# MycroftAI/mimic3

Hardware: AMD Instinct MI355X
Metric: 22.05 kHz audio samples/sec/node (en_UK/apope_low VITS hot path: run + int16, host ids in -> host int16 out) (higher is better)
Workload: dtype f32 (dense convs: operands split exactly into 3 x bf16, 6 bf16-MFMA products per multiply-add, f32 accumulate; f32 in / f32 out, parity at the f32 tolerances)

## Files before the change

### mimic3_amd/csrc/engine.cpp

```cpp
#include "engine.h"

#include <algorithm>
#include <cmath>
#include <cstdlib>
#include <cstring>
#include <fstream>
#include <sstream>

namespace m355 {

namespace {
struct Reader {
    const unsigned char* p;
    size_t n, pos = 0;
    void need(size_t k) const {
        if (pos + k > n) throw EngineError(MI355VITS_ERR_FORMAT, "weight container truncated");
    }
    template <typename T> T get() {
        need(sizeof(T));
        T v;
        memcpy(&v, p + pos, sizeof(T));
        pos += sizeof(T);
        return v;
    }
// ... 1080 lines not shown
        conv("convflow.proj", cw(p + ".proj"), a);
        {
            ProfScope ps(prof_, "spline");
            launch_spline_inverse(d_z2_, ch0, d_theta_, d_len_, B, Tx, c.dp_num_bins, c.dp_tail_bound,
                                  1.0f / sqrtf((float)H), stream_);
        }
    }
    ch0 ^= 1;
    {
        ProfScope ps(prof_, "durations");
        launch_durations(d_z2_, ch0, model_->ea_m[0], model_->ea_logs[0], d_len_, d_forced_, B, Tx, d_scales_, d_logw_, d_wceil_,
                         d_cum_, d_ylen_, stream_);
    }
    tap("logw", d_logw_, {B, 1, Tx});
}

static const char* stage_label(int i, const char* const (&t)[4]) { return t[std::min(i, 3)]; }

void Engine::coupling_layer(int j, int B, int Ty) {
    const mi355vits_config& c = cfg_;
    const int H = c.hidden_channels, I = c.inter_channels, half = I / 2;
    const long zbs = (long)I * Ty, hbs = (long)H * Ty;
    const bool rev = ((c.flow_n_flows - 1 - j) % 2) == 0;
    float* x0 = d_z_ + (rev ? (long)half * Ty : 0);
    float* x1 = d_z_ + (rev ? 0 : (long)half * Ty);
    ConvArgs pre;
    pre.x = x0; pre.x_bs = zbs; pre.x_ld = Ty;
    pre.y = d_fh_; pre.y_bs = hbs; pre.y_ld = Ty;
    pre.out_len = d_ylen_;
    pre.B = B; pre.T = Ty;
    conv("flow.pre", cw(S("flow.%d.pre", j)), pre);
    float* hcur = d_fh_;
    float* hnext = d_fh2_;
    for (int l = 0; l < c.flow_wn_layers; ++l) {
        int dil = 1;
        for (int q = 0; q < l; ++q) dil *= c.flow_wn_dilation_rate;
        const ConvW& win = cw(S("flow.%d.in.%d", j, l));
        const ConvW& wrs = cw(S("flow.%d.rs.%d", j, l));
        const float* cond_l = d_cond_flow_.empty() ? nullptr : d_cond_flow_[j] + (long)l * 2 * H;
        const bool wn_b3 = sw_.wn_b3 && math_on_bf16(kmath()) && win.packed_b3s != NO_OFF && wrs.packed_b3s != NO_OFF &&
                           conv1d_b3_supported(win.Cin, win.Cout, win.K, dil, Ty) && !sw_.force_generic;
        const bool fused = !sw_.force_generic && !sw_.no_fused_wn && !wn_b3;
        const bool b3 = fused && math_on_bf16(kmath()) && win.packed_b3w != NO_OFF && wrs.packed_b3s != NO_OFF &&
                        wn_layer_b3_supported(H, win.K, dil);
        if (b3 || (fused && wn_layer_fused_supported(H, win.K, dil))) {
            const bool h2 = b3 && math_ == MATH_F16X2 && win.packed_h2s != NO_OFF && wrs.packed_h2s != NO_OFF;
            WnArgs w;
            w.h_in = hcur; w.h_out = hnext; w.h_bs = hbs; w.h_ld = Ty;
            w.skip = d_fskip_; w.s_bs = hbs; w.s_ld = Ty;
            w.w_in = P(h2 ? win.packed_h2s : (b3 ? win.packed_b3w : win.packed)); w.b_in = P(win.bias);
            w.w_rs = P(h2 ? wrs.packed_h2s : (b3 ? wrs.packed_b3s : wrs.packed)); w.b_rs = P(wrs.bias);
            w.cond = cond_l; w.cond_bs = 2L * H * c.flow_wn_layers;
            w.len = d_ylen_;
            w.B = B; w.H = H; w.T = Ty; w.K = win.K; w.dil = dil; w.Crs = wrs.Cout; w.skip_init = (l == 0);
            if (b3) w.math = h2 ? (int)MATH_F16X2 : kmath();
            const double fl = 2.0 * B * (double)Ty * H * ((double)win.Cout * win.K + wrs.Cout);
            ProfScope ps(prof_, b3 ? "flow.wn_layer_b3" : "flow.wn_layer", fl, 4.0 * B * (double)Ty * H * 4);
            if (b3) launch_wn_layer_b3(w, stream_);
            else launch_wn_layer(w, stream_);
            if (wrs.Cout == 2 * H) std::swap(hcur, hnext);
            continue;
        }
        ConvArgs in;
        in.x = hcur; in.x_bs = hbs; in.x_ld = Ty;
        in.y = d_fu_; in.y_bs = hbs; in.y_ld = Ty;
        in.epi = EPI_GATE; in.H = H; in.dil = dil;
        if (cond_l) {
            in.cond = cond_l;
            in.cond_bs = 2L * H * c.flow_wn_layers;
        }
        in.B = B; in.T = Ty;
        if (wn_b3) in.math = kmath();
        conv("flow.in_gate", win, in);
        ConvArgs rs;
        rs.x = d_fu_; rs.x_bs = hbs; rs.x_ld = Ty;
        rs.y = hcur; rs.y_bs = hbs; rs.y_ld = Ty;
        rs.y2 = d_fskip_; rs.y2_bs = hbs; rs.y2_ld = Ty;
        rs.epi = EPI_RESSKIP; rs.H = H; rs.skip_init = (l == 0);
        rs.out_len = d_ylen_;
        rs.B = B; rs.T = Ty;
        if (wn_b3) rs.math = kmath();
        conv("flow.res_skip", wrs, rs);
    }
    ConvArgs post;
    post.x = d_fskip_; post.x_bs = hbs; post.x_ld = Ty;
    post.y = x1; post.y_bs = zbs; post.y_ld = Ty;
    post.res = x1; post.res_bs = zbs; post.res_ld = Ty; post.res_sub = 1;
    post.in_len = d_ylen_; post.out_len = d_ylen_;
    post.B = B; post.T = Ty;
    conv("flow.post_couple", cw(S("flow.%d.post", j)), post);
}

ConvArgs Engine::rb2_conv_args(int i, int j, int m, int B, int ch, long T) const {
    const mi355vits_config& c = cfg_;
    float* const pp[2] = {d_bufB_, d_bufT_};
    const bool last = (m == c.resblock_n_dilations[j] - 1);
    const float* src = m == 0 ? d_bufA_ : pp[(m - 1) & 1];
    ConvArgs a;
    a.x = src; a.x_bs = (long)ch * T; a.x_ld = (int)T;
    a.y = last ? d_bufC_ : pp[m & 1]; a.y_bs = (long)ch * T; a.y_ld = (int)T;
    a.res = src; a.res_bs = (long)ch * T; a.res_ld = (int)T;
    a.in_slope = 0.1f; a.dil = c.resblock_dilations[j * MI355VITS_MAX_STAGES + m];
    a.in_len = d_slen_ + (long)(i + 1) * B;
    if (last) { a.out_scale = 1.0f / c.n_resblock_kernels; a.accumulate = (j > 0); }
    a.B = B; a.T = (int)T;
    return a;
// ... 450 lines not shown
```

### mimic3_amd/csrc/kernels.h

```cpp
#pragma once
#include "hipx.h"

#include <vector>

namespace m355 {

struct Profiler;

enum ConvEpilogue { EPI_STD = 0, EPI_GATE = 1, EPI_RESSKIP = 2 };

struct ConvArgs {
    const float* x = nullptr; long x_bs = 0; int x_ld = 0;
    float* y = nullptr;       long y_bs = 0; int y_ld = 0;
    const float* w = nullptr;
    const float* wb3 = nullptr;
    int math = 0;
    const float* bias = nullptr;
    const float* cond = nullptr; long cond_bs = 0;
    const float* res = nullptr; long res_bs = 0; int res_ld = 0;
    float* y2 = nullptr; long y2_bs = 0; int y2_ld = 0;
    const int* in_len = nullptr;
    const int* in_len_host = nullptr;
    int nvalid = 0;
    int rb_loop = 0;
// ... 67 lines not shown
    const float* bias[MRF_MAX_RB][2] = {};
    int k[MRF_MAX_RB] = {}, d1[MRF_MAX_RB] = {}, d2[MRF_MAX_RB] = {};
    int nrb = 0;
    const int* len = nullptr;
    int B = 1, C = 0, T = 0;
    int R = 0, ldx = 0, ld1 = 0, vec = 0;
    float out_scale = 0.0f;
    int ablate = 0;
    int seg = 0;
    unsigned* clk = nullptr;
    const int* len_host = nullptr;
    int nvalid = 0;
    int prio = 0;
};
bool mrf_fused_supported(int C, int nrb, const int* k, const int* d1, const int* d2);
void launch_mrf_fused(MrfArgs a, hipStream_t s);
inline int mrf_stage_halo(int nrb, const int* k, const int* d1, const int* d2) {
    int R = 0;
    for (int j = 0; j < nrb; ++j) {
        const int r = (k[j] - 1) / 2 * d1[j] + (k[j] - 1) / 2 * d2[j];
        R = R > r ? R : r;
    }
    return R;
}
struct MrfPlan { int width = 0, halo = 0, x_ring = 0, x1_ring = 0; };
bool mrf_fused_plan(int C, int nrb, const int* k, const int* d1, const int* d2, MrfPlan* out);
bool mrf_p_plan(int C, int nrb, const int* k, const int* d1, const int* d2, MrfPlan* out);
bool mrf_s_plan(int C, int nrb, const int* k, const int* d1, const int* d2, MrfPlan* out);
size_t p16_packed_words(int Cout, int Cin, int K);
void pack_conv_weights_p16(const float* w, int Cout, int Cin, int K, uint32_t* out);
bool mrf_p_supported(int C, int nrb, const int* k, const int* d1, const int* d2);
int mrf_valid_items(const int* len_host, const int* len_dev, int B, int T, int block, int extra = 0);
void launch_mrf_p(MrfArgs a, hipStream_t s);
bool mrf_s_supported(int C, int nrb, const int* k, const int* d1, const int* d2);
int mrf_s_segment(int C, int B, int T, int cus, const int* len_host = nullptr);
void launch_mrf_s(MrfArgs a, hipStream_t s);
bool rb_conv_supported(const ConvArgs& a);
void launch_rb_conv(ConvArgs a, hipStream_t s);
void pack_conv_weights_p16n(const float* w, int Cout, int Cin, int K, uint32_t* out);
bool ups_pl_supported(const ConvArgs& a);
void launch_ups_pl(ConvArgs a, hipStream_t s);
int current_device_cu_count();
void set_max_dynamic_lds(const void* fn, int bytes);

struct WnArgs {
    const float* h_in = nullptr; float* h_out = nullptr; long h_bs = 0; int h_ld = 0;
    float* skip = nullptr; long s_bs = 0; int s_ld = 0;
    const float* w_in = nullptr;
    const float* b_in = nullptr;
    const float* w_rs = nullptr;
    const float* b_rs = nullptr;
    const float* cond = nullptr; long cond_bs = 0;
    const int* len = nullptr;
    int B = 1, H = 0, T = 0, K = 1, dil = 1, Crs = 0, skip_init = 0;
    int ldx = 0, vec = 0;
    int ablate = 0;
    int math = 0;
};
bool wn_layer_fused_supported(int H, int K, int dil);
void launch_wn_layer(WnArgs a, hipStream_t s);
bool wn_layer_b3_supported(int H, int K, int dil);
void launch_wn_layer_b3(WnArgs a, hipStream_t s);
int wn_layer_b3_column_tiles(const WnArgs& a);
int wn_layer_geometry(const WnArgs& a);

void launch_conv_post_tanh(const float* x, long x_bs, int x_ld, const float* w, int Cin, int K, int B, int L,
                           const int* valid_len, float* audio, long audio_bs, unsigned* peak_bits, hipStream_t s);
void launch_pcm16(const float* audio, long audio_bs, const unsigned* peak_bits, const int* valid_len, int B, int L,
                  int16_t* pcm, long pcm_bs, hipStream_t s, const double* volumes = nullptr);
enum PackEncoding { PACK_ENC_S16 = 0, PACK_ENC_ULAW = 1, PACK_ENC_ALAW = 2, PACK_ENC_F32 = 3 };
constexpr int pack_bytes_per_sample(int enc) { return enc == PACK_ENC_S16 ? 2 : enc == PACK_ENC_F32 ? 4 : 1; }
inline size_t pack_capacity_bytes(int enc, long total) { return ((size_t)total * pack_bytes_per_sample(enc) + 15) & ~size_t(15); }
enum { PACK_SEG_OFFSET = 0, PACK_SEG_ROW = 1, PACK_SEG_LENGTH = 2, PACK_SEG_SKIP = 3 };
constexpr int pack_seg_scale_row(bool trimmed) { return trimmed ? 4 : 3; }
constexpr int pack_seg_rows(bool trimmed, bool normalised) { return pack_seg_scale_row(trimmed) + (normalised ? 1 : 0); }
constexpr int pack_seg_curve_row(bool trimmed) { return pack_seg_scale_row(trimmed) + 1; }
constexpr int pack_seg_rows(bool trimmed, bool normalised, bool curved) { return pack_seg_rows(trimmed, normalised) + (curved ? 1 : 0); }
void launch_pack(int enc, const float* audio, long audio_bs, const unsigned* peak_bits, const double* volumes, const int* seg, int n,
                 uint8_t* out, long total, hipStream_t s, bool trimmed, bool normalised, const float* curve = nullptr);
enum { PACK_ENT_OFFSET = 0, PACK_ENT_ROW = 1, PACK_ENT_LENGTH = 2, PACK_ENT_SKIP = 3, PACK_ENT_ENC = 4, PACK_ENT_SCALE = 5, PACK_ENT_ROWS = 6 };
enum { PACK_ENT_SCALED = 4, PACK_ENT_CURVED = 8 };
enum { PACK_ENT_CURVE = 6 };
constexpr int pack_ent_rows(bool curved) { return curved ? PACK_ENT_ROWS + 1 : PACK_ENT_ROWS; }
enum { PACK_STREAM_BEGIN = 0, PACK_STREAM_DATA = 1, PACK_STREAM_END = 2, PACK_STREAM_ENC = 3, PACK_STREAM_HEADER = 4, PACK_STREAM_WORDS = 20 };
constexpr long PACK_STREAMS_ITEM_BYTES = 256L * 16;
inline size_t pack_streams_capacity(long n_bytes) { return ((size_t)n_bytes + 15) & ~size_t(15); }
inline size_t pack_streams_table_words(int n_entries, int n_streams, bool curved = false) {
    return (size_t)pack_ent_rows(curved) * n_entries + (size_t)PACK_STREAM_WORDS * n_streams;
}
void launch_pack_streams(const float* audio, long audio_bs, const unsigned* peak_bits, const double* volumes, const int* tab, int n_entries,
                         int n_streams, uint8_t* out, long n_bytes, hipStream_t s, const float* curve = nullptr);
void launch_g711_encode(int law, const int16_t* in, long n, uint8_t* out, hipStream_t s);

constexpr int FLAC_BLOCK = 4096;
constexpr int FLAC_SLOT_BYTES = 8208;
constexpr int FLAC_HEADER_BYTES = 42;
constexpr int FLAC_MAX_RATE = 0xfffff;
constexpr long FLAC_MAX_FRAME_NUMBER = 0x1fffff;
struct FlacJob {
    const int16_t* src;
    long n;
    int first_frame;
    int slot0;
};
inline long flac_frames(long n) { return (n + FLAC_BLOCK - 1) / FLAC_BLOCK; }
inline size_t flac_out_capacity(long n_frames, long total) { return (16 * (size_t)n_frames + 2 * (size_t)total + 15) & ~size_t(15); }
void launch_flac_frames(const FlacJob* jobs, int n_jobs, long n_frames, int rate, uint8_t* slots, int* sizes, hipStream_t s);
void launch_flac_gather(const uint8_t* slots, int* sizes, long long* offsets, long n_frames, uint8_t* out, hipStream_t s);
// ... 170 lines not shown
```

### mimic3_amd/csrc/kernels_wn.cpp

```cpp
#include "kernels.h"
#include "b3.h"

namespace m355 {

template <int CP>
__device__ __forceinline__ void wn_mfma2(f32x16& acc0, f32x16& acc1, const float* __restrict__ wp0,
                                         const float* __restrict__ wp1, const float* __restrict__ xw, int LD, int K, int dil) {
    static_assert(CP % 8 == 0, "channel pairs per tap must be a multiple of 8");
    const int ld2 = 2 * LD;
    float r0[8], r1[8];
    MI355_UNROLL
    for (int u = 0; u < 4; ++u) { r0[u] = wp0[u * 64]; r1[u] = wp1[u * 64]; }
    float bb[2];
    bb[0] = xw[0];
    const float* g0 = wp0;
    const float* g1 = wp1;
    for (int k = 0; k < K; ++k) {
        MI355_UNROLL
        for (int cp0 = 0; cp0 < CP; cp0 += 8) {
            const float* base = xw + k * dil + cp0 * ld2;
            const bool last = (k == K - 1) && (cp0 + 8 == CP);
            const float* nbase = last ? base : ((cp0 + 8 < CP) ? base + 8 * ld2 : xw + (k + 1) * dil);
            const float* h0 = last ? g0 - 8 * 64 : g0;
            const float* h1 = last ? g1 - 8 * 64 : g1;
            MI355_UNROLL
            for (int u = 0; u < 8; ++u) {
                const float a0 = r0[u], a1 = r1[u];
                r0[(u + 4) & 7] = (u < 4) ? g0[(u + 4) * 64] : h0[(u + 4) * 64];
                r1[(u + 4) & 7] = (u < 4) ? g1[(u + 4) * 64] : h1[(u + 4) * 64];
                bb[(u + 1) & 1] = (u < 7) ? base[(u + 1) * ld2] : nbase[0];
                acc0 = MFMA_32x32x2_F32(a0, bb[u & 1], acc0);
                acc1 = MFMA_32x32x2_F32(a1, bb[u & 1], acc1);
                SCHED_FENCE();
            }
            g0 += 8 * 64;
            g1 += 8 * 64;
        }
    }
}

template <int NP>
__global__ __launch_bounds__(64 * NP) MIN_WAVES_PER_SIMD(NP > 1 ? 5 : 1) void k_wn_layer(WnArgs a) {
    constexpr int H = 32 * NP;
    constexpr int CP = H / 2;
    constexpr int T_B = 32;
    DYN_SMEM(float, smem);
    const int LDX = a.ldx;
    float* X = smem;
    float* U = smem;
    const int tid = threadIdx.x, lane = tid & 63, p = WAVE_UNIFORM(tid >> 6);
    const int brow = lane >> 5, bcol = lane & 31;
    const int b = blockIdx.y;
    const int t0 = blockIdx.x * T_B;
    int len = a.len ? a.len[b] : a.T;
// ... 285 lines not shown
        for (int r = 0; r < 16; ++r) sp[(long)((r & 3) + 8 * (r >> 2)) * a.s_ld] = a.skip_init ? acc[r] : old[r] + acc[r];
    };
    if (two) {
        f32x16 acc[MT];
        const float* wp[MT];
        MI355_UNROLL
        for (int m = 0; m < MT; ++m) {
            const int q = MT * w + m;
            MI355_UNROLL
            for (int r = 0; r < 16; ++r) acc[m][r] = a.b_rs[32 * q + (r & 3) + 8 * (r >> 2) + 4 * brow];
            wp[m] = a.w_rs + (long)q * CP * 64 + lane;
        }
        if (!(LAB_ABLATE(a) & 1)) wn_mfma_b4<MT, CP>(acc, wp, U, 32, 1, 0);
        MI355_UNROLL
        for (int m = 0; m < MT; ++m) finish(acc[m], MT * w + m, hres[m]);
    } else if (NW == 12) {
        if (w < 6) {
            f32x16 a1[1];
            const float* w1[1] = {a.w_rs + (long)w * CP * 64 + lane};
            MI355_UNROLL
            for (int r = 0; r < 16; ++r) a1[0][r] = a.b_rs[32 * w + (r & 3) + 8 * (r >> 2) + 4 * brow];
            if (!(LAB_ABLATE(a) & 1)) wn_mfma_b4<1, CP>(a1, w1, U, 32, 1, 0);
            finish(a1[0], w, hres[0]);
        }
    } else {
        const int nq = w < 2 ? 2 : 1;
        f32x16 acc[2];
        const float* wp[2];
        MI355_UNROLL
        for (int m = 0; m < 2; ++m) {
            const int q = m == 0 ? w : w + 4;
            const int qq = q < 6 ? q : w;
            MI355_UNROLL
            for (int r = 0; r < 16; ++r) acc[m][r] = a.b_rs[32 * qq + (r & 3) + 8 * (r >> 2) + 4 * brow];
            wp[m] = a.w_rs + (long)qq * CP * 64 + lane;
        }
        if (!(LAB_ABLATE(a) & 1)) {
            if (nq == 2) {
                wn_mfma_b4<2, CP>(acc, wp, U, 32, 1, 0);
            } else {
                f32x16 a1[1] = {acc[0]};
                const float* w1[1] = {wp[0]};
                wn_mfma_b4<1, CP>(a1, w1, U, 32, 1, 0);
                acc[0] = a1[0];
            }
        }
        finish(acc[0], w, hres[0]);
        if (nq == 2) finish(acc[1], w + 4, hres[0]);
    }
}

constexpr int WNB_H = 192, WNB_NG = WNB_H / 16;
constexpr int WNB_RING = 4;
constexpr int WNB_EPI = 1;
#if defined(MI355_LAB) && !defined(MI355_EMU)
#define WN_TS_DECL() long long wn_ts[7] = {0, 0, 0, 0, 0, 0, 0}
#define WN_TS(i) do { if (a.ablate & 64) wn_ts[i] = __builtin_readcyclecounter(); } while (0)
#define WN_TS_END()                                                                                                                  \
    do {                                                                                                                             \
        if ((a.ablate & 64) && blockIdx.x == 3 && blockIdx.y == 5 && threadIdx.x == 0) {                                            \
            __builtin_amdgcn_s_waitcnt(0);                                                                                           \
            wn_ts[6] = __builtin_readcyclecounter();                                                                                 \
            printf("wn phases (cycles): stage %lld inconv %lld rawstore %lld gate+planes %lld rs %lld epilogue %lld total %lld\n", wn_ts[1] - wn_ts[0], \
                   wn_ts[2] - wn_ts[1], wn_ts[3] - wn_ts[2], wn_ts[4] - wn_ts[3], wn_ts[5] - wn_ts[4], wn_ts[6] - wn_ts[5], wn_ts[6] - wn_ts[0]);   \
        }                                                                                                                            \
    } while (0)
#else
#define WN_TS_DECL() ((void)0)
#define WN_TS(i) ((void)0)
#define WN_TS_END() ((void)0)
#endif


template <bool W1, int NT, bool H2, int RA, int EP>
__device__ __forceinline__ void wn_layer_b3_body(const WnArgs& a) {
    constexpr int MW = 3, NWV = 4, NTH = 256;
    static_assert(!(W1 && H2), "one reduced-operand variant at a time");
    constexpr int H = WNB_H, T_B = 32 * NT, NG = WNB_NG;
    constexpr int NP = H2 ? 2 : 3, GW = H2 ? 128 : 192;
    constexpr float ACC = H2 ? F16X2_ACC_SCALE : 1.0f, UNACC = H2 ? 1.0f / F16X2_ACC_SCALE : 1.0f;
    DYN_SMEM(float, smem);
    uint4* planes = reinterpret_cast<uint4*>(smem);
    const int tid = threadIdx.x, lane = tid & 63, w = WAVE_UNIFORM(tid >> 6);
    const int brow = lane >> 5, bcol = lane & 31;
    const int b = blockIdx.y;
    const int t0 = blockIdx.x * T_B;
    int len = a.len ? a.len[b] : a.T;
    if (len > a.T) len = a.T;
    if (t0 >= len) return;
    const int pad = (a.K - 1) / 2 * a.dil;
    const int tlo = t0 - pad;
    const int ts = tlo >= 0 ? (tlo & ~3) : -(((-tlo) + 3) & ~3);
    const int toff = tlo - ts;
    const int LD = a.ldx;
    WN_TS_DECL();
    WN_TS(0);
    const int PS = NG * 2 * LD;
    const bool two = a.Crs == 2 * H;

    if (!(LAB_ABLATE(a) & 2)) stage_planes<NG, NG, H2>(a.h_in + (long)b * a.h_bs, a.h_ld, LD, ts, len, 1.0f, planes, PS, tid, NTH);
    __syncthreads();
    WN_TS(1);

    const float* condp = a.cond ? a.cond + (long)b * a.cond_bs : a.b_in;
    const float cond_on = a.cond ? 1.0f : 0.0f;
    {
        f32x16 acc[MW][NT];
        const uint4* wp[MW];
        MI355_UNROLL
        for (int i = 0; i < MW; ++i) {
            const int q = w + NWV * i;
            MI355_UNROLL
            for (int r = 0; r < 16; ++r) {
                const int c = (r < 8 ? 0 : H) + 16 * q + (r & 3) + 8 * ((r >> 2) & 1) + 4 * brow;
                const float v = (a.b_in[c] + cond_on * condp[c]) * ACC;
                MI355_UNROLL
                for (int j = 0; j < NT; ++j) acc[i][j][r] = v;
            }
            wp[i] = reinterpret_cast<const uint4*>(a.w_in) + (long)q * a.K * NG * GW + lane;
        }
        if (!(LAB_ABLATE(a) & 1)) {
            if constexpr (H2) h2_chunk<MW, NT, NG, NT>(acc, wp, planes + brow * LD + bcol + toff, PS, LD, a.K, NG, a.dil);
            else if constexpr (RA > 2 && NT >= 4) b3_chunk_lean_ra<MW, NT, NG, W1, RA>(acc, wp, planes + brow * LD + bcol + toff, PS, LD, a.K, NG, a.dil);
            else if constexpr (RA > 2) b3_chunk_ra<MW, NT, NG, NT, W1, RA>(acc, wp, planes + brow * LD + bcol + toff, PS, LD, a.K, NG, a.dil);
            else b3_chunk<MW, NT, NG, NT, W1>(acc, wp, planes + brow * LD + bcol + toff, PS, LD, a.K, NG, a.dil);
        }
        __syncthreads();
        WN_TS(2);
        WN_TS(3);
        constexpr int PSU0 = NG * 2 * T_B;
        MI355_UNROLL
        for (int i = 0; i < MW; ++i)
            MI355_UNROLL
            for (int j = 0; j < NT; ++j) {
                float u[8];
                MI355_UNROLL
                for (int e = 0; e < 8; ++e) u[e] = wn_gate_f(acc[i][j][e] * UNACC, acc[i][j][e + 8] * UNACC);
                const int idx = (2 * (w + NWV * i) + brow) * T_B + 32 * j + bcol;
                if constexpr (H2) {
                    uint4 h4, m4;
                    split2_pk(u[0] * F16X2_X_SCALE, u[1] * F16X2_X_SCALE, h4.x, m4.x);
                    split2_pk(u[2] * F16X2_X_SCALE, u[3] * F16X2_X_SCALE, h4.y, m4.y);
// ... 98 lines not shown
                    for (int j = 0; j < NT; ++j) acc[i][j] = a2[i][j];
            }
        }
        if constexpr (H2) {
            MI355_UNROLL
            for (int i = 0; i < MW; ++i)
                MI355_UNROLL
                for (int j = 0; j < NT; ++j)
                    MI355_UNROLL
                    for (int r = 0; r < 16; ++r) acc[i][j][r] *= UNACC;
        }
    }
    WN_TS(5);
    if ((LAB_ABLATE(a) & 4) && acc[0][0][0] != 1.2345f) return;
    auto store_tile = [&](int i, int j, const float (&old)[16]) {
        const int t = t0 + j * 32 + bcol;
        if (!valid[i] || t >= a.T) return;
        const bool live = t < len || !to_h[i];
        MI355_UNROLL
        for (int r = 0; r < 16; ++r) dst[i][(long)((r & 3) + 8 * (r >> 2) + 4 * brow) * ldr[i] + t] = live ? old[r] + acc[i][j][r] : 0.0f;
    };
    if constexpr (EP == 0) {
        load_tile(0, 0, old[0]);
        MI355_UNROLL
        for (int k = 0; k < MW * NT; ++k) {
            if (k + 1 < MW * NT) load_tile((k + 1) / NT, (k + 1) % NT, old[(k + 1) & 1]);
            SCHED_FENCE();
            store_tile(k / NT, k % NT, old[k & 1]);
            SCHED_FENCE();
        }
    } else {
        auto store_tile_b = [&](int i, int j, const float (&o)[16]) MI355_INLINE_LAMBDA {
            const int t = t0 + j * 32 + bcol;
            const bool live = t < len || !to_h[i];
            const BufRsrc rs = buf_rsrc(dst[i]);
            const unsigned row4 = 4u * (unsigned)ldr[i];
            const unsigned vo = (valid[i] && t < a.T) ? (unsigned)(4 * brow) * row4 + 4u * (unsigned)t : BUF_OOB;
            MI355_UNROLL
            for (int r = 0; r < 16; ++r) buf_store_f32(rs, vo, (unsigned)((r & 3) + 8 * (r >> 2)) * row4, live ? o[r] + acc[i][j][r] : 0.0f);
        };
        MI355_UNROLL
        for (int k = 0; k < EPA && k < MW * NT; ++k) load_tile_b(k / NT, k % NT, old[k]);
        MI355_UNROLL
        for (int k = 0; k < MW * NT; ++k) {
            if (k + EPA < MW * NT) load_tile_b((k + EPA) / NT, (k + EPA) % NT, old[(k + EPA) % EPR]);
            SCHED_FENCE();
            store_tile_b(k / NT, k % NT, old[k % EPR]);
            SCHED_FENCE();
        }
    }
    WN_TS_END();
}

template <bool W1, int NT, bool H2 = false, int RA = 2, int EP = 0>
__global__ __launch_bounds__(256) void k_wn_layer_b3(WnArgs a) {
    wn_layer_b3_body<W1, NT, H2, RA, EP>(a);
}

bool wn_layer_b3_supported(int H, int K, int dil) {
    return H == WNB_H && (K % 2) == 1 && K >= 1 && dil >= 1 && (K - 1) * dil <= 24;
}

int wn_layer_b3_column_tiles(const WnArgs& a) {
    const char* nt_s = lab_getenv("MI355VITS_WN_B3_NT");
    const long nwg3 = (long)((a.T + 95) / 96) * a.B;
    int nt = nt_s ? atoi(nt_s) : (nwg3 < 128 ? 1 : 3);
    if (!nt_s && nt == 3 && a.math != MATH_F16X2) {
        const long cus = current_device_cu_count();
        const long nwg4 = (long)((a.T + 127) / 128) * a.B;
        if ((double)((nwg4 + cus - 1) / cus) * 1.28 < (double)((nwg3 + cus - 1) / cus)) nt = 4;
    }
    if (nt == 4 && (a.math == MATH_F16X2 || ((long)a.h_ld * 128 >= 0x7fffffffL || (long)a.s_ld * 128 >= 0x7fffffffL || (a.K - 1) * a.dil > 8))) nt = 3;
    return nt;
}

void launch_wn_layer_b3(WnArgs a, hipStream_t s) {
    if (a.T <= 0 || a.B <= 0) return;
    if (!wn_layer_b3_supported(a.H, a.K, a.dil)) throw std::runtime_error("wn_layer_b3: unsupported shape");
    static const int ablate = lab_getenv("MI355VITS_WN_ABLATE") ? atoi(lab_getenv("MI355VITS_WN_ABLATE")) : 0;
    a.ablate = ablate;
    a.vec = (a.h_ld % 4 == 0) && (a.h_bs % 4 == 0) && (reinterpret_cast<uintptr_t>(a.h_in) % 16 == 0);
    const int nt = wn_layer_b3_column_tiles(a);
    const int tb = 32 * nt;
    a.ldx = (tb + (a.K - 1) * a.dil + 3 + 3) & ~3;
    const size_t shmem = (size_t)3 * WNB_NG * 2 * a.ldx * 16;
    dim3 grid((a.T + tb - 1) / tb, a.B);
    auto go = [&](auto kfn) {
#ifndef MI355_EMU
        set_max_dynamic_lds(reinterpret_cast<const void*>(kfn), 160 * 1024);
#endif
        LAUNCH_KERNEL(kfn, grid, dim3(256), shmem, s, a);
    };
    if (nt == 4 && a.math != MATH_F16X2) {
        if (a.math == MATH_BF16W) go(k_wn_layer_b3<true, 4, false, WNB_RING, 1>);
        else go(k_wn_layer_b3<false, 4, false, WNB_RING, 1>);
    } else if (nt == 1) {
        if (a.math == MATH_F16X2) go(k_wn_layer_b3<false, 1, true>);
        else if (a.math == MATH_BF16W) go(k_wn_layer_b3<true, 1>);
        else go(k_wn_layer_b3<false, 1>);
    } else {
        int epi = WNB_EPI;
        if (const char* f = lab_getenv("MI355VITS_WN_EPI")) epi = atoi(f);
        if ((long)a.h_ld * 128 >= 0x7fffffffL || (long)a.s_ld * 128 >= 0x7fffffffL) epi = 0;
        if (a.math == MATH_F16X2) go(k_wn_layer_b3<false, 3, true>);
        else if (a.math == MATH_BF16W) go(k_wn_layer_b3<true, 3>);
        else if (epi == 1) go(k_wn_layer_b3<false, 3, false, WNB_RING, 1>);
        else go(k_wn_layer_b3<false, 3, false, WNB_RING>);
    }
}

bool wn_layer_fused_supported(int H, int K, int dil) {
    return (H == 32 || H == 192) && (K % 2) == 1 && K >= 1 && dil >= 1 && (size_t)H * (32 + (K - 1) * dil + 8) * 4 <= 48 * 1024;
}

int wn_layer_geometry(const WnArgs& a) {
    const char* six_s = lab_getenv("MI355VITS_WN_SIX_WAVES");
    const int six_env = six_s ? atoi(six_s) : -1;
    const long nwg = (long)((a.T + 31) / 32) * a.B;
    return six_env >= 0 ? six_env : (nwg < 128 ? 2 : (nwg < 512 ? 1 : 0));
}

void launch_wn_layer(WnArgs a, hipStream_t s) {
    if (a.T <= 0 || a.B <= 0) return;
    if (!wn_layer_fused_supported(a.H, a.K, a.dil)) throw std::runtime_error("wn_layer: unsupported shape");
    a.ldx = (32 + (a.K - 1) * a.dil + 3 + 3) & ~3;
    static const int ablate = lab_getenv("MI355VITS_WN_ABLATE") ? atoi(lab_getenv("MI355VITS_WN_ABLATE")) : 0;
    a.ablate = ablate;
    a.vec = (a.h_ld % 4 == 0) && (a.h_bs % 4 == 0) && (reinterpret_cast<uintptr_t>(a.h_in) % 16 == 0);
    const size_t shmem = (size_t)a.H * a.ldx * sizeof(float);
    dim3 grid((a.T + 31) / 32, a.B);
    const int geom = wn_layer_geometry(a);
    const size_t sh4 = (size_t)a.H * (a.ldx > 64 ? a.ldx : 64) * sizeof(float);
    if (a.H == 192 && geom == 0) {
        LAUNCH_KERNEL(k_wn_layer_h192<4>, grid, dim3(256), sh4, s, a);
    } else if (a.H == 192 && geom == 2) {
        LAUNCH_KERNEL(k_wn_layer_h192<12>, grid, dim3(768), sh4, s, a);
    } else if (a.H == 192) {
        auto k = k_wn_layer<6>;
        LAUNCH_KERNEL(k, grid, dim3(384), shmem, s, a);
    } else {
        auto k = k_wn_layer<1>;
        LAUNCH_KERNEL(k, grid, dim3(64), shmem, s, a);
    }
}

}
```

### mimic3_amd/csrc/lab_api.cpp

```cpp
#include "c_api_internal.h"
#include "mi355vits_lab.h"

extern "C" {

int mi355vits_probe_weights(mi355vits_handle h, double out[8]) {
    if (!h || !out) return MI355VITS_ERR_INVALID;
    std::lock_guard<std::mutex> lk(h->eng->mu);
    return guarded(h, [&] { h->eng->probe_weights(out); });
}

int mi355vits_test_conv1d(int device, const mi355vits_conv_test* t) {
    return guarded(nullptr, [&] {
        if (!t || !t->x || !t->w || !t->y) throw EngineError(MI355VITS_ERR_INVALID, "null argument");
        HIP_CHECK(hipSetDevice(device));
        const size_t nx = (size_t)t->B * t->Cin * t->T, ny = (size_t)t->B * t->Cout * t->T;
        const size_t nw = (size_t)t->Cout * t->Cin * t->K;
        DevBuf dx(nx * 4), dy(ny * 4), dw(nw * 4), db(t->Cout * 4), dres(ny * 4), dil(t->B * 4), dol(t->B * 4);
        std::vector<float> packed;
        HIP_CHECK(hipMemcpy(dx.p, t->x, nx * 4, hipMemcpyHostToDevice));
        HIP_CHECK(hipMemcpy(dy.p, t->y, ny * 4, hipMemcpyHostToDevice));
        ConvArgs a;
        a.x = dx.as<float>(); a.x_bs = (long)t->Cin * t->T; a.x_ld = t->T;
        a.y = dy.as<float>(); a.y_bs = (long)t->Cout * t->T; a.y_ld = t->T;
        a.B = t->B; a.Cin = t->Cin; a.Cout = t->Cout; a.T = t->T; a.K = t->K; a.dil = t->dilation;
// ... 538 lines not shown
            } else {
                dwr = upload(w_rs.data(), w_rs.size() * 4);
            }
            ConvArgs in;
            in.x = dh.as<float>(); in.x_bs = hbs; in.x_ld = T;
            in.y = du.as<float>(); in.y_bs = hbs; in.y_ld = T;
            in.epi = EPI_GATE; in.H = H; in.dil = dil;
            if (t->cond) { in.cond = dc.as<float>(); in.cond_bs = 2L * H; }
            in.B = B; in.T = T;
            in.fixed_rule = 1; in.Cin = H; in.Cout = 2 * H; in.K = K; in.bias = dbi.as<float>(); in.pad = (K * dil - dil) / 2;
            in.w = dwi->as<float>(); in.math = MATH_F32;
            ConvArgs rs;
            rs.x = du.as<float>(); rs.x_bs = hbs; rs.x_ld = T;
            rs.y = dh.as<float>(); rs.y_bs = hbs; rs.y_ld = T;
            rs.y2 = dsk.as<float>(); rs.y2_bs = hbs; rs.y2_ld = T;
            rs.epi = EPI_RESSKIP; rs.H = H; rs.skip_init = t->skip_init != 0;
            rs.out_len = dl.as<int>();
            rs.B = B; rs.T = T;
            rs.fixed_rule = 1; rs.Cin = H; rs.Cout = Crs; rs.K = 1; rs.bias = dbr.as<float>(); rs.pad = 0;
            rs.w = dwr->as<float>(); rs.math = MATH_F32;
            if (mfma_in) launch_conv1d_mfma(in, nullptr);
            else launch_conv1d_generic(in, nullptr);
            if (mfma_rs) launch_conv1d_mfma(rs, nullptr);
            else launch_conv1d_generic(rs, nullptr);
            h_result = dh.as<float>();
        } else {
            if (t->impl == 1) {
                std::vector<float> pi(mfma_packed_floats(2 * H, H, K), 0.0f), pr(mfma_packed_floats(Crs, H, 1), 0.0f);
                pack_conv_weights_mfma_mode(w_in.data(), 2 * H, H, K, EPI_GATE, pi.data());
                pack_conv_weights_mfma_mode(w_rs.data(), Crs, H, 1, EPI_STD, pr.data());
                dwi = upload(pi.data(), pi.size() * 4);
                dwr = upload(pr.data(), pr.size() * 4);
            } else {
                const size_t row = (size_t)H * K;
                std::vector<float> wg(w_in.size());
                for (int q = 0; q < 2 * H / 32; ++q)
                    for (int r = 0; r < 32; ++r) {
                        const int src = (r < 16 ? 0 : H) + 16 * q + (r & 15);
                        memcpy(wg.data() + ((size_t)32 * q + r) * row, w_in.data() + (size_t)src * row, row * sizeof(float));
                    }
                std::vector<uint32_t> bi(bf16x3_packed_words_mode(2 * H, H, K, EPI_STD)), br(bf16x3_packed_words_mode(Crs, H, 1, EPI_STD));
                pack_conv_weights_bf16x3_mode(wg.data(), 2 * H, H, K, EPI_STD, 1, bi.data());
                pack_conv_weights_bf16x3_mode(w_rs.data(), Crs, H, 1, EPI_STD, 1, br.data());
                dwi = upload(bi.data(), bi.size() * 4);
                dwr = upload(br.data(), br.size() * 4);
            }
            WnArgs w;
            w.h_in = dh.as<float>(); w.h_out = dho.as<float>(); w.h_bs = hbs; w.h_ld = T;
            w.skip = dsk.as<float>(); w.s_bs = hbs; w.s_ld = T;
            w.w_in = dwi->as<float>(); w.b_in = dbi.as<float>();
            w.w_rs = dwr->as<float>(); w.b_rs = dbr.as<float>();
            if (t->cond) { w.cond = dc.as<float>(); w.cond_bs = 2L * H; }
            w.len = dl.as<int>();
            w.B = B; w.H = H; w.T = T; w.K = K; w.dil = dil; w.Crs = Crs; w.skip_init = t->skip_init != 0;
            if (t->impl == 2) { w.math = MATH_BF16X3; launch_wn_layer_b3(w, nullptr); }
            else launch_wn_layer(w, nullptr);
        }
        HIP_CHECK(hipDeviceSynchronize());
        HIP_CHECK(hipGetLastError());
        if (t->impl != 0 || Crs == 2 * H) HIP_CHECK(hipMemcpy(t->h_out, h_result, n * 4, hipMemcpyDeviceToHost));
        HIP_CHECK(hipMemcpy(t->skip, dsk.p, n * 4, hipMemcpyDeviceToHost));
    });
}

int mi355vits_lab_wn_plan(int B, int T, int K, int dilation, int32_t* b3_tile, int32_t* f32_geometry) {
    return guarded(nullptr, [&] {
        if (B < 1 || T < 1 || K < 1 || (K % 2) == 0 || dilation < 1) throw EngineError(MI355VITS_ERR_INVALID, "bad shape");
        WnArgs w;
        w.B = B; w.H = 192; w.T = T; w.K = K; w.dil = dilation; w.h_ld = w.s_ld = T; w.math = MATH_BF16X3;
        if (b3_tile) {
            if (!wn_layer_b3_supported(w.H, K, dilation)) throw EngineError(MI355VITS_ERR_INVALID, "shape not supported by the fused split-bf16 layer");
            *b3_tile = 32 * wn_layer_b3_column_tiles(w);
        }
        if (f32_geometry) *f32_geometry = wn_layer_geometry(w);
    });
}

static bool mrf_test_plan(int impl, int C, int nrb, const int32_t* k, const int32_t* d1, const int32_t* d2, MrfPlan* p) {
    if (nrb < 1 || nrb > MRF_MAX_RB || !k || !d1 || !d2) return false;
    int kk[MRF_MAX_RB], a1[MRF_MAX_RB], a2[MRF_MAX_RB];
    for (int j = 0; j < nrb; ++j) { kk[j] = k[j]; a1[j] = d1[j]; a2[j] = d2[j]; }
    return impl == 0 ? mrf_fused_plan(C, nrb, kk, a1, a2, p) : impl == 1 ? mrf_p_plan(C, nrb, kk, a1, a2, p) : impl == 2 ? mrf_s_plan(C, nrb, kk, a1, a2, p) : false;
}

int mi355vits_test_mrf_stage(int device, const mi355vits_mrf_test* t) {
    return guarded(nullptr, [&] {
        if (!t || !t->x || !t->len || !t->y) throw EngineError(MI355VITS_ERR_INVALID, "null argument");
        const int B = t->B, C = t->C, T = t->T, nrb = t->nrb;
        if (B < 1 || C < 1 || T < 1 || nrb < 1 || nrb > MRF_MAX_RB || !(t->out_scale >= 0.0f)) throw EngineError(MI355VITS_ERR_INVALID, "bad shape");
        if ((long)C * T * 4 >= 0x7fffffffL || (long)B * C * T >= 0x7fffffffL / 4) throw EngineError(MI355VITS_ERR_INVALID, "tensor too large for the hook");
        for (int j = 0; j < nrb; ++j)
            for (int q = 0; q < 2; ++q)
                if (!t->w[j][q] || !t->bias[j][q]) throw EngineError(MI355VITS_ERR_INVALID, "null weight or bias");
        for (int b = 0; b < B; ++b)
            if (t->len[b] < 0 || t->len[b] > T) throw EngineError(MI355VITS_ERR_INVALID, "len out of range");
        if (t->impl < 0 || t->impl > 2) throw EngineError(MI355VITS_ERR_INVALID, "impl must be 0, 1 or 2");
        if (t->impl == 0 ? (t->math != MATH_F32 && t->math != MATH_BF16X3) : t->math != MATH_BF16X3)
            throw EngineError(MI355VITS_ERR_INVALID, "math mode: MATH_F32 or MATH_BF16X3 for impl 0, MATH_BF16X3 for impl 1 and 2");
        MrfPlan plan;
        if (!mrf_test_plan(t->impl, C, nrb, t->k, t->d1, t->d2, &plan)) throw EngineError(MI355VITS_ERR_INVALID, "stage not supported by the chosen kernel");
        if (t->impl == 2 && (t->seg < plan.width || t->seg % plan.width != 0)) throw EngineError(MI355VITS_ERR_INVALID, "seg must be a positive multiple of the sweep's step");
        HIP_CHECK(hipSetDevice(device));
        const size_t n = (size_t)B * C * T;
        DevBuf dx(n * 4), dy(n * 4), dl((size_t)B * 4);
        HIP_CHECK(hipMemcpy(dx.p, t->x, n * 4, hipMemcpyHostToDevice));
        HIP_CHECK(hipMemcpy(dy.p, t->y, n * 4, hipMemcpyHostToDevice));
// ... 193 lines not shown
```

Before: 783.8 million.

## Make fused split-bf16 WN layer kernel persistent over valid tiles

Turns the wide (NT=3/4) fused WaveNet flow layer kernel into a persistent kernel. A grid capped at the CU count loops over only the valid (row, time-tile) items, counted on the host from sequence lengths, and items are grouped per XCD for locality. The goal is to stop launching blocks for padded time tiles that exit early, and to balance work across CUs for batches with ragged lengths. In exchange it adds a per-item row-locate loop and a __syncthreads between tiles, and the per-block LDS setup is no longer paid only once per launch.

```diff
diff --git a/mimic3_amd/csrc/engine.cpp b/mimic3_amd/csrc/engine.cpp
--- a/mimic3_amd/csrc/engine.cpp
+++ b/mimic3_amd/csrc/engine.cpp
@@ -1156,6 +1156,7 @@
             w.w_rs = P(h2 ? wrs.packed_h2s : (b3 ? wrs.packed_b3s : wrs.packed)); w.b_rs = P(wrs.bias);
             w.cond = cond_l; w.cond_bs = 2L * H * c.flow_wn_layers;
             w.len = d_ylen_;
+            w.len_host = h_ylen_.data();
             w.B = B; w.H = H; w.T = Ty; w.K = win.K; w.dil = dil; w.Crs = wrs.Cout; w.skip_init = (l == 0);
             if (b3) w.math = h2 ? (int)MATH_F16X2 : kmath();
             const double fl = 2.0 * B * (double)Ty * H * ((double)win.Cout * win.K + wrs.Cout);
diff --git a/mimic3_amd/csrc/kernels.h b/mimic3_amd/csrc/kernels.h
--- a/mimic3_amd/csrc/kernels.h
+++ b/mimic3_amd/csrc/kernels.h
@@ -143,8 +143,10 @@
     const float* b_rs = nullptr;
     const float* cond = nullptr; long cond_bs = 0;
     const int* len = nullptr;
+    const int* len_host = nullptr;
     int B = 1, H = 0, T = 0, K = 1, dil = 1, Crs = 0, skip_init = 0;
     int ldx = 0, vec = 0;
+    int nvalid = 0;
     int ablate = 0;
     int math = 0;
 };
diff --git a/mimic3_amd/csrc/kernels_wn.cpp b/mimic3_amd/csrc/kernels_wn.cpp
--- a/mimic3_amd/csrc/kernels_wn.cpp
+++ b/mimic3_amd/csrc/kernels_wn.cpp
@@ -1,5 +1,6 @@
 #include "kernels.h"
 #include "b3.h"
+#include <type_traits>
 
 namespace m355 {
 
@@ -391,6 +392,11 @@
 
 constexpr int WNB_H = 192, WNB_NG = WNB_H / 16;
 constexpr int WNB_RING = 4;
+#if defined(MI355_LAB) || defined(MI355_EMU)
+constexpr bool WN_LAB_FORMS = true;
+#else
+constexpr bool WN_LAB_FORMS = false;
+#endif
 constexpr int WNB_EPI = 1;
 #if defined(MI355_LAB) && !defined(MI355_EMU)
 #define WN_TS_DECL() long long wn_ts[7] = {0, 0, 0, 0, 0, 0, 0}
@@ -411,8 +417,8 @@
 #endif
 
 
-template <bool W1, int NT, bool H2, int RA, int EP>
-__device__ __forceinline__ void wn_layer_b3_body(const WnArgs& a) {
+template <bool W1, int NT, bool H2, int RA, int EP, int PF>
+__device__ __forceinline__ void wn_layer_b3_tile(const WnArgs& a, const int b, const int t0, const int len, const int lane, const int w) {
     constexpr int MW = 3, NWV = 4, NTH = 256;
     static_assert(!(W1 && H2), "one reduced-operand variant at a time");
     constexpr int H = WNB_H, T_B = 32 * NT, NG = WNB_NG;
@@ -420,13 +426,8 @@
     constexpr float ACC = H2 ? F16X2_ACC_SCALE : 1.0f, UNACC = H2 ? 1.0f / F16X2_ACC_SCALE : 1.0f;
     DYN_SMEM(float, smem);
     uint4* planes = reinterpret_cast<uint4*>(smem);
-    const int tid = threadIdx.x, lane = tid & 63, w = WAVE_UNIFORM(tid >> 6);
+    const int tid = 64 * w + lane;
     const int brow = lane >> 5, bcol = lane & 31;
-    const int b = blockIdx.y;
-    const int t0 = blockIdx.x * T_B;
-    int len = a.len ? a.len[b] : a.T;
-    if (len > a.T) len = a.T;
-    if (t0 >= len) return;
     const int pad = (a.K - 1) / 2 * a.dil;
     const int tlo = t0 - pad;
     const int ts = tlo >= 0 ? (tlo & ~3) : -(((-tlo) + 3) & ~3);
@@ -631,9 +632,61 @@
     WN_TS_END();
 }
 
-template <bool W1, int NT, bool H2 = false, int RA = 2, int EP = 0>
+template <bool W1, int NT, bool H2, int RA, int EP, int PF>
+__device__ __forceinline__ void wn_layer_b3_body(const WnArgs& a) {
+    constexpr int T_B = 32 * NT;
+    const int tid = threadIdx.x, lane = tid & 63, w = WAVE_UNIFORM(tid >> 6);
+    auto row_len = [&](int bb) MI355_INLINE_LAMBDA {
+        const int ln = a.len ? a.len[bb] : a.T;
+        return ln > a.T ? a.T : ln;
+    };
+    if constexpr (PF == 0) {
+        const int b = blockIdx.y;
+        const int t0 = blockIdx.x * T_B;
+        const int len = row_len(b);
+        if (t0 >= len) return;
+        wn_layer_b3_tile<W1, NT, H2, RA, EP, 0>(a, b, t0, len, lane, w);
+    } else {
+        const int nitems = a.nvalid;
+        const int nblk = gridDim.x, ngrp = nblk < 8 ? nblk : 8, xcd = blockIdx.x % ngrp, slot = blockIdx.x / ngrp;
+        const int per_xcd = (nitems + ngrp - 1) / ngrp, nslot = (nblk + ngrp - 1 - xcd) / ngrp;
+        const int item_end = (xcd + 1) * per_xcd < nitems ? (xcd + 1) * per_xcd : nitems;
+        struct Cursor { int r, base, nv; };
+        auto locate = [&](int v, Cursor& c) MI355_INLINE_LAMBDA {
+            while (v >= c.base + c.nv && c.r + 1 < a.B) {
+                c.base += c.nv;
+                ++c.r;
+                const int ln = row_len(c.r);
+                c.nv = ln > 0 ? (ln + T_B - 1) / T_B : 0;
+            }
+            c.r = WAVE_UNIFORM(c.r);
+            c.base = WAVE_UNIFORM(c.base);
+            c.nv = WAVE_UNIFORM(c.nv);
+        };
+        Cursor cur;
+        cur.r = 0;
+        cur.base = 0;
+        {
+            const int ln = row_len(0);
+            cur.nv = ln > 0 ? (ln + T_B - 1) / T_B : 0;
+        }
+        for (int item = xcd * per_xcd + slot; item < item_end; item += nslot) {
+            locate(item, cur);
+            int lane_o = lane, w_o = w;
+            OPAQUE_V(lane_o);
+            OPAQUE_S(w_o);
+            const int b = cur.r, t0 = WAVE_UNIFORM((item - cur.base) * T_B);
+            const int len = WAVE_UNIFORM(row_len(b));
+            if (t0 >= len) continue;
+            wn_layer_b3_tile<W1, NT, H2, RA, EP, PF>(a, b, t0, len, lane_o, w_o);
+            __syncthreads();
+        }
+    }
+}
+
+template <bool W1, int NT, bool H2 = false, int RA = 2, int EP = 0, int PF = 0>
 __global__ __launch_bounds__(256) void k_wn_layer_b3(WnArgs a) {
-    wn_layer_b3_body<W1, NT, H2, RA, EP>(a);
+    wn_layer_b3_body<W1, NT, H2, RA, EP, PF>(a);
 }
 
 bool wn_layer_b3_supported(int H, int K, int dil) {
@@ -664,15 +717,36 @@
     a.ldx = (tb + (a.K - 1) * a.dil + 3 + 3) & ~3;
     const size_t shmem = (size_t)3 * WNB_NG * 2 * a.ldx * 16;
     dim3 grid((a.T + tb - 1) / tb, a.B);
+    bool persist = nt != 1;
+    if (WN_LAB_FORMS && persist) {
+        if (const char* f = lab_getenv("MI355VITS_WN_PERSIST")) persist = atoi(f) != 0;
+    }
+    if (persist) {
+        a.nvalid = mrf_valid_items(a.len_host, a.len, a.B, a.T, tb);
+        if (a.nvalid <= 0) return;
+        const int cus = current_device_cu_count();
+        grid = dim3((unsigned)(a.nvalid < cus ? a.nvalid : cus));
+    }
     auto go = [&](auto kfn) {
 #ifndef MI355_EMU
         set_max_dynamic_lds(reinterpret_cast<const void*>(kfn), 160 * 1024);
 #endif
         LAUNCH_KERNEL(kfn, grid, dim3(256), shmem, s, a);
     };
+    auto wide = [&](auto W1c, auto NTc, auto H2c, auto RAc, auto EPc) {
+        constexpr bool W1 = decltype(W1c)::value, H2 = decltype(H2c)::value;
+        constexpr int NT = decltype(NTc)::value, RA = decltype(RAc)::value, EP = decltype(EPc)::value;
+        if constexpr (WN_LAB_FORMS) {
+            if (!persist) { go(k_wn_layer_b3<W1, NT, H2, RA, EP, 0>); return; }
+        }
+        go(k_wn_layer_b3<W1, NT, H2, RA, EP, 1>);
+    };
+    using std::integral_constant;
+    using Tr = std::true_type;
+    using Fa = std::false_type;
     if (nt == 4 && a.math != MATH_F16X2) {
-        if (a.math == MATH_BF16W) go(k_wn_layer_b3<true, 4, false, WNB_RING, 1>);
-        else go(k_wn_layer_b3<false, 4, false, WNB_RING, 1>);
+        if (a.math == MATH_BF16W) wide(Tr{}, integral_constant<int, 4>{}, Fa{}, integral_constant<int, WNB_RING>{}, integral_constant<int, 1>{});
+        else wide(Fa{}, integral_constant<int, 4>{}, Fa{}, integral_constant<int, WNB_RING>{}, integral_constant<int, 1>{});
     } else if (nt == 1) {
         if (a.math == MATH_F16X2) go(k_wn_layer_b3<false, 1, true>);
         else if (a.math == MATH_BF16W) go(k_wn_layer_b3<true, 1>);
@@ -681,10 +755,10 @@
         int epi = WNB_EPI;
         if (const char* f = lab_getenv("MI355VITS_WN_EPI")) epi = atoi(f);
         if ((long)a.h_ld * 128 >= 0x7fffffffL || (long)a.s_ld * 128 >= 0x7fffffffL) epi = 0;
-        if (a.math == MATH_F16X2) go(k_wn_layer_b3<false, 3, true>);
-        else if (a.math == MATH_BF16W) go(k_wn_layer_b3<true, 3>);
-        else if (epi == 1) go(k_wn_layer_b3<false, 3, false, WNB_RING, 1>);
-        else go(k_wn_layer_b3<false, 3, false, WNB_RING>);
+        if (a.math == MATH_F16X2) wide(Fa{}, integral_constant<int, 3>{}, Tr{}, integral_constant<int, 2>{}, integral_constant<int, 0>{});
+        else if (a.math == MATH_BF16W) wide(Tr{}, integral_constant<int, 3>{}, Fa{}, integral_constant<int, 2>{}, integral_constant<int, 0>{});
+        else if (epi == 1) wide(Fa{}, integral_constant<int, 3>{}, Fa{}, integral_constant<int, WNB_RING>{}, integral_constant<int, 1>{});
+        else wide(Fa{}, integral_constant<int, 3>{}, Fa{}, integral_constant<int, WNB_RING>{}, integral_constant<int, 0>{});
     }
 }
 
diff --git a/mimic3_amd/csrc/lab_api.cpp b/mimic3_amd/csrc/lab_api.cpp
--- a/mimic3_amd/csrc/lab_api.cpp
+++ b/mimic3_amd/csrc/lab_api.cpp
@@ -614,6 +614,7 @@
             w.w_rs = dwr->as<float>(); w.b_rs = dbr.as<float>();
             if (t->cond) { w.cond = dc.as<float>(); w.cond_bs = 2L * H; }
             w.len = dl.as<int>();
+            w.len_host = t->len;
             w.B = B; w.H = H; w.T = T; w.K = K; w.dil = dil; w.Crs = Crs; w.skip_init = t->skip_init != 0;
             if (t->impl == 2) { w.math = MATH_BF16X3; launch_wn_layer_b3(w, nullptr); }
             else launch_wn_layer(w, nullptr);
```

After: 776.7 million. About the same (-0.9%).
